# robustrobotics/multi_view_stereonet

Hardware: AMD Instinct MI355X
Metric: depthmaps/sec at 512x256, 64 hypotheses, 2 src views; L1 vs ref (higher is better)
Workload: dtype f32; 1 GPU; GTA-SfM-shaped 512x256, D=64 hypotheses, 2 source views, cost-volume filter + 5 refiners; global_batch=256, parallelism=dp1 (independent images, all-gather of metric rows)

## Files before the change

### include/mvsn_hip.h

```cpp
#ifndef MVSN_HIP_H
#define MVSN_HIP_H

#include <stddef.h>
#include <stdint.h>

#ifdef __cplusplus
extern "C" {
#endif

#define MVSN_ABI_VERSION 6

#define MVSN_E_BADARG (-1)
#define MVSN_E_TOOLARGE (-2)
#define MVSN_E_WORKSPACE (-3)

typedef void *mvsn_stream_t;

int mvsn_abi_version(void);
const char *mvsn_last_error(void);

int mvsn_plane_sweep_setup(const float *T_right_in_left, const float *K_lvl0, const float *K_lvl4,
                           int n_chains, int rows4, int cols4, int num_idepth_samples,
                           float *idepth_samples, float *H_lvl4, float *H_inc, float *H_lvl0_plane0,
                           float *baseline, mvsn_stream_t stream);
// ... 104 lines not shown
                              long spatial, float *out, mvsn_stream_t stream);
int mvsn_groupnorm_lrelu_apply_records(const float *x, const float *records, int tiles, const float *gamma,
                                       const float *beta, const float *residual, const float *r_stats,
                                       const float *r_gamma, const float *r_beta, int n, long spatial, float *out,
                                       mvsn_stream_t stream);

int mvsn_conv_to1_supported(int rows, int cols);
int mvsn_conv_to1(const float *in, const float *weight, const float *bias, const float *prior, const float *fx,
                  int n, int depth, int rows, int cols, int kd, float *out, mvsn_stream_t stream);
int mvsn_conv_to1_volume_norm(const float *in_raw, const float *in_stats, const float *in_gamma, const float *in_beta,
                              const float *weight, const float *bias, int n, int depth, int rows, int cols, float *out,
                              mvsn_stream_t stream);
int mvsn_conv_to1_block(const float *in_raw, const float *in_stats, const float *in_gamma, const float *in_beta,
                        const float *in_residual, const float *weight, const float *bias, const float *prior,
                        const float *fx, int n, int rows, int cols, float *out, mvsn_stream_t stream);
int mvsn_conv_to1_block_records(const float *in_raw, const float *in_records, int tiles, const float *in_gamma,
                                const float *in_beta, const float *in_residual, const float *weight, const float *bias,
                                const float *prior, const float *fx, int n, int rows, int cols, float *out,
                                mvsn_stream_t stream);

int mvsn_soft_argmin(const float *cost, const float *idepth_samples, int n, int num_idepth_samples,
                     int pixels, float *idepth, mvsn_stream_t stream);

int mvsn_soft_argmin_confidence(const float *cost, const float *idepth_samples, int n, int num_idepth_samples,
                                int pixels, float *idepth, float *confidence, mvsn_stream_t stream);
int mvsn_confidence_fuse_sources(const float *confidence, int n_sources, int batch, int pixels, float *out,
                                 mvsn_stream_t stream);
int mvsn_confidence_mask(const float *confidence, const uint8_t *valid, long count, float min_confidence,
                         uint8_t *out, mvsn_stream_t stream);
int mvsn_fusion_gather(const float *maps, const int *view, const int *pixel, int n_views, long pixels_per_view,
                       long count, float *out, mvsn_stream_t stream);

int mvsn_channel_l2_norm(const float *x, int n, int channels, long pixels, float *out, mvsn_stream_t stream);
int mvsn_idepth_scale(const float *prior, const float *fx, int n, long pixels, float *out, mvsn_stream_t stream);
int mvsn_refiner_epilogue(const float *prior, const float *fx, const float *delta, int n, long pixels, float *out,
                          mvsn_stream_t stream);

int mvsn_upsample_bilinear(const float *in, int n, int channels, int rows_in, int cols_in, int rows_out,
                           int cols_out, float *out, mvsn_stream_t stream);
int mvsn_upsample_prior(const float *in, const float *fx, int n, int rows_in, int cols_in, int rows_out, int cols_out,
                        float *out, float *out_scaled, mvsn_stream_t stream);
int mvsn_upsample_mask(const uint8_t *in, int n, int channels, int rows_in, int cols_in, int rows_out,
                       int cols_out, uint8_t *out, mvsn_stream_t stream);

int mvsn_area_downsample(const float *in, int n, int channels, int rows_in, int cols_in, float *out,
                         mvsn_stream_t stream);

int mvsn_image_pyramid_supported(int rows, int cols, int levels);
int mvsn_image_pyramid(const float *in, int n, int channels, int rows, int cols, int levels, float *const *out_levels,
                       mvsn_stream_t stream);
int mvsn_prepare_cameras(const float *K, const float *T_right_in_left, int batch, int n_sources, int levels,
                         const int *level_sizes_dev, float *K_pyr, float *T_normalised, float *T_inverse_normalised,
                         float *baseline, mvsn_stream_t stream);

int mvsn_fuse_sources(const float *raw, const float *refined, const float *baseline, const uint8_t *mask,
                      int n_sources, int batch, int num_idepth_samples, int pixels, int refined_aliases_raw,
                      float *raw_out, float *refined_out, uint8_t *mask_out, mvsn_stream_t stream);

int mvsn_idepth_reproject_blocks(int pixels);
int mvsn_idepth_reproject(const float *K, const float *T_other_in_this, const float *idepth, const float *other_idepth,
                          const uint8_t *other_mask, int batch, int rows, int cols, float *idepth_in_other,
                          float *other_sampled, uint8_t *other_mask_sampled, uint8_t *invalid, float *uv,
                          float *absdiff_partials, mvsn_stream_t stream);
int mvsn_occlusion_mask(const float *idepth_in_other, const float *other_sampled, const uint8_t *invalid,
                        const float *absdiff_partials, int batch, int pixels, uint8_t *mask, mvsn_stream_t stream);
int mvsn_masked_l1(const float *a, const float *b, const uint8_t *skip_a, const uint8_t *skip_b, long n, int accumulate,
                   float *loss, mvsn_stream_t stream);

typedef struct {
  const float *in[3];
  int channels[3], sample_mod[3];
  const float *block_scale;
  int scale_mod, scale_block;
  int head_chunks, n_blocks;
  int dilation[6];
  const float *weights, *params;
  int tail_mode;
  const float *prior, *fx;
  int fx_mod;
  float *out;
} mvsn_tower_desc;
int mvsn_tower_16x32(const mvsn_tower_desc *desc, int n_samples, mvsn_stream_t stream);

int mvsn_depth_metrics_blocks(long pixels);
int mvsn_depth_metrics(const float *idepth_est, const float *depth_true, const float *baseline, int batch, long pixels,
                       float min_depth, float max_depth, double *partials, double *rows, mvsn_stream_t stream);

size_t mvsn_fusion_workspace_bytes(int n_ref, int n_slots, int rows, int cols);
int mvsn_fusion_consistency(const float *depth, const uint8_t *valid, const float *K, const float *T_cam_in_world,
                            const int *ref_views, const int *neighbours, int n_views, int n_ref, int n_slots, int rows,
                            int cols, float max_reproj_px, float max_rel_depth, int min_consistent, float *fused_depth,
                            uint8_t *count, int64_t *total, void *workspace, size_t workspace_bytes,
                            mvsn_stream_t stream);
int mvsn_fusion_emit(const float *fused_depth, const float *images, const int *ref_views, int n_ref, int rows, int cols,
                     int n_slots, const void *workspace, size_t workspace_bytes, long capacity, float *points,
                     uint8_t *colors, int *view, int *pixel, mvsn_stream_t stream);

#define MVSN_VOXEL_STATUS_RANGE 1
#define MVSN_VOXEL_STATUS_TABLE 2
size_t mvsn_voxel_workspace_bytes(long n);
int mvsn_voxel_assign(const float *points, long n, float voxel_size, float inv_voxel_size, float origin_x,
                      float origin_y, float origin_z, int64_t *result, void *workspace, size_t workspace_bytes,
                      mvsn_stream_t stream);
int mvsn_voxel_merge(const float *points, const uint8_t *colors, long n, float voxel_size, float inv_voxel_size,
                     float origin_x, float origin_y, float origin_z, void *workspace, size_t workspace_bytes,
                     long capacity, void *accumulators, float *out_points, uint8_t *out_colors, int *count,
                     int64_t *first, int64_t *inverse, mvsn_stream_t stream);

int mvsn_depth_normals(const float *depth, const uint8_t *valid, const float *K, const float *T_cam_in_world,
                       int n_views, int rows, int cols, float max_rel_step, float *normals, mvsn_stream_t stream);
int mvsn_normals_gather(const float *normals, const int *view, const int *pixel, int n_views, long pixels_per_view,
                        long count, float *out, mvsn_stream_t stream);
int mvsn_voxel_normals(const float *normals, const int64_t *inverse, long n, long m, void *accumulators, float *out,
                       mvsn_stream_t stream);

#define MVSN_CLOUD_STATUS_RANGE 1
#define MVSN_CLOUD_STATUS_TABLE 2
size_t mvsn_cloud_workspace_bytes(long n_target);
int mvsn_cloud_index_build(const float *target, long n, float cell, float inv_cell, int64_t *status, void *workspace,
                           size_t workspace_bytes, mvsn_stream_t stream);
int mvsn_cloud_nearest(const float *query, long nq, float inv_cell, float r2, const void *workspace,
                       size_t workspace_bytes, long n_target, float *dist2, int64_t *index, int *within,
                       mvsn_stream_t stream);

int mvsn_tsdf_camera_batch(void);
int mvsn_tsdf_integrate(const float *depth, const uint8_t *valid, const float *weights, const float *images,
                        const float *K, const float *T_cam_in_world, int n_views, int rows, int cols, int nx, int ny,
                        int nz, float voxel_size, float origin_x, float origin_y, float origin_z, float trunc,
                        float min_depth, float *sdf_sum, float *weight, float *color_sum, mvsn_stream_t stream);
size_t mvsn_tsdf_workspace_bytes(int nx, int ny, int nz);
int mvsn_tsdf_classify(const float *sdf_sum, const float *weight, int nx, int ny, int nz, float min_weight,
                       int64_t *result, void *workspace, size_t workspace_bytes, mvsn_stream_t stream);
int mvsn_tsdf_extract(const float *sdf_sum, const float *weight, const float *color_sum, int nx, int ny, int nz,
                      float voxel_size, float origin_x, float origin_y, float origin_z, float min_weight,
                      const void *workspace, size_t workspace_bytes, long n_vertices, long n_quads, float *vertices,
                      float *normals, uint8_t *colors, int64_t *faces, int64_t *cell, mvsn_stream_t stream);

size_t mvsn_tsdf_raycast_workspace_bytes(int nx, int ny, int nz);
int mvsn_tsdf_raycast(const float *sdf_sum, const float *weight, const float *color_sum, int nx, int ny, int nz,
                      float voxel_size, float origin_x, float origin_y, float origin_z, const float *K,
                      const float *T_cam_in_world, int n_views, int rows, int cols, float min_weight, float min_depth,
                      float max_depth, float step, void *workspace, size_t workspace_bytes, float *depth,
                      float *normals, float *colors, float *weight_out, mvsn_stream_t stream);

int mvsn_copy(void *dst, const void *src, size_t nbytes, mvsn_stream_t stream);
int mvsn_copy_many(void *const *dst, const void *const *src, const size_t *nbytes, int count, mvsn_stream_t stream);
int mvsn_gather_focal(const float *const *K_pyr, int levels, int batch, float *fx, mvsn_stream_t stream);
int mvsn_gather_strided(const float *src, int count, long stride, float *dst, mvsn_stream_t stream);

int mvsn_debug_set_band_flags(int flags);

int mvsn_debug_set_wino_rowphase(int mode);

int mvsn_debug_wino_plan(const mvsn_conv_desc *desc, int carrying, int out[8]);

int mvsn_debug_conv_plan(const mvsn_conv_desc *desc, int mode, int out[8]);

int mvsn_selftest_mfma(mvsn_stream_t stream);

#ifdef __cplusplus
}
#endif
#endif
```

### multi_view_stereonet_amd/_native.py

```python
import ctypes
import os
from ctypes import c_char_p, c_int, c_long, c_size_t, c_void_p, POINTER, Structure

import torch

_LIB_PATH = os.path.join(os.path.dirname(os.path.abspath(__file__)), "libmvsn_hip.so")
_lib = None


class ConvDesc(Structure):
    _fields_ = [("n", c_int), ("c_in", c_int), ("c_out", c_int), ("depth", c_int), ("rows", c_int),
                ("cols", c_int), ("kd", c_int), ("kh", c_int), ("kw", c_int), ("stride", c_int),
                ("dilation", c_int), ("precision", c_int)]


class ApplyJob(Structure):
    _fields_ = [("x", c_void_p), ("stats", c_void_p), ("gamma", c_void_p), ("beta", c_void_p),
                ("residual", c_void_p), ("r_stats", c_void_p), ("r_gamma", c_void_p), ("r_beta", c_void_p),
                ("out", c_void_p), ("n", c_int), ("reverse", c_int), ("spatial", c_long)]


class TowerDesc(Structure):
    _fields_ = [("inp", c_void_p * 3), ("channels", c_int * 3), ("sample_mod", c_int * 3), ("block_scale", c_void_p),
                ("scale_mod", c_int), ("scale_block", c_int), ("head_chunks", c_int), ("n_blocks", c_int),
                ("dilation", c_int * 6), ("weights", c_void_p), ("params", c_void_p), ("tail_mode", c_int),
                ("prior", c_void_p), ("fx", c_void_p), ("fx_mod", c_int), ("out", c_void_p)]


CONV_FP32, CONV_BF16X3, CONV_FP32_WINO, CONV_BF16 = 0, 1, 2, 3
CHAIN_AUTO, CHAIN_DIRECT, CHAIN_WINOGRAD, CHAIN_STEPWISE, CHAIN_BANDED = 0, 1, 2, 3, 4
ABI_VERSION = 6


SIGNATURES = {
    "mvsn_abi_version": (c_int, []),
    "mvsn_last_error": (c_char_p, []),
    "mvsn_plane_sweep_setup": (c_int, [c_void_p] * 3 + [c_int] * 4 + [c_void_p] * 5 + [c_void_p]),
    "mvsn_plane_sweep_setup_sources": (c_int, [POINTER(c_void_p), c_int, c_void_p, c_void_p] + [c_int] * 4 + [c_void_p] * 5 + [c_void_p]),
    "mvsn_plane_sweep_setup_path": (c_int, [c_void_p, c_void_p, c_int, c_int]),
    "mvsn_gather_focal": (c_int, [POINTER(c_void_p), c_int, c_int, c_void_p, c_void_p]),
    "mvsn_homography_warp": (c_int, [c_void_p] * 2 + [c_int] * 5 + [c_void_p] * 2 + [c_void_p]),
    "mvsn_feature_refiner_packed_floats": (c_size_t, []),
    "mvsn_pack_feature_refiner": (c_int, [c_void_p] * 11 + [c_void_p]),
    "mvsn_incremental_cost_volume_workspace_bytes": (c_size_t, [c_int] * 3),
    "mvsn_incremental_cost_volume_form": (c_int, [c_int] * 2),
    "mvsn_incremental_cost_volume_form_for": (c_int, [c_int] * 3),
    "mvsn_incremental_cost_volume_workspace_bytes_for": (c_size_t, [c_int] * 5),
    "mvsn_incremental_cost_volume_resolve": (c_int, [c_int] * 7 + [POINTER(c_size_t * 8)]),
    "mvsn_incremental_cost_volume_status_offset": (c_size_t, [c_int] * 3),
    "mvsn_incremental_cost_volume_banded_groups": (c_int, [c_int] * 3),
    "mvsn_incremental_cost_volume": (c_int, [c_void_p] * 6 + [c_int] * 5 + [c_void_p] * 4 + [c_size_t, c_int, c_void_p]),
    "mvsn_incremental_cost_volume_repair_workspace_bytes": (c_size_t, [c_int] * 3),
    "mvsn_incremental_cost_volume_guarded": (c_int, [c_void_p] * 6 + [c_int] * 5 + [c_void_p] * 4 +
                                             [c_size_t, c_int, c_void_p, c_size_t, c_void_p, c_void_p]),
    "mvsn_incremental_cost_volume_bf16": (c_int, [c_void_p] * 6 + [c_int] * 5 + [c_void_p] * 4 +
                                          [c_size_t, c_int, c_void_p, c_size_t, c_void_p, c_void_p]),
    "mvsn_conv_bf16x3_supported": (c_int, [POINTER(ConvDesc)]),
    "mvsn_conv_forward_bf16_storage": (c_int, [c_void_p, c_void_p, c_int, c_void_p, c_void_p, c_void_p, c_void_p, c_void_p,
                                               c_void_p, c_int, c_void_p, c_void_p]),
    "mvsn_conv_winograd_supported": (c_int, [POINTER(ConvDesc)]),
    "mvsn_conv_packed_floats": (c_size_t, [POINTER(ConvDesc)]),
    "mvsn_conv_pack_weights": (c_int, [POINTER(ConvDesc), c_void_p, c_void_p, c_void_p]),
    "mvsn_conv_num_tiles": (c_int, [POINTER(ConvDesc)]),
    "mvsn_conv_forward": (c_int, [POINTER(ConvDesc)] + [c_void_p] * 10 + [c_void_p]),
    "mvsn_conv_forward_blocks": (c_int, [POINTER(ConvDesc), c_void_p, POINTER(c_int), c_int] + [c_void_p] * 4 + [c_void_p]),
    "mvsn_conv_forward_carry": (c_int, [POINTER(ConvDesc)] + [c_void_p] * 8 + [POINTER(ApplyJob), POINTER(c_int), c_void_p]),
    "mvsn_groupnorm_finalize": (c_int, [c_void_p, c_int, c_int, c_void_p, c_void_p]),
    "mvsn_groupnorm_finalize_split_workspace_bytes": (c_size_t, [c_int, c_int]),
    "mvsn_groupnorm_finalize_split": (c_int, [c_void_p, c_int, c_int, c_void_p, c_void_p, c_size_t, c_void_p]),
    "mvsn_groupnorm_lrelu_apply": (c_int, [c_void_p] * 5 + [c_int, c_long, c_void_p, c_void_p]),
    "mvsn_groupnorm_lrelu_add2": (c_int, [c_void_p] * 8 + [c_int, c_long, c_void_p, c_void_p]),
    "mvsn_conv_to1_block": (c_int, [c_void_p] * 9 + [c_int] * 3 + [c_void_p, c_void_p]),
    "mvsn_debug_set_band_flags": (c_int, [c_int]),
    "mvsn_debug_set_wino_rowphase": (c_int, [c_int]),
    "mvsn_debug_wino_plan": (c_int, [POINTER(ConvDesc), c_int, POINTER(c_int * 8)]),
    "mvsn_debug_conv_plan": (c_int, [POINTER(ConvDesc), c_int, POINTER(c_int * 8)]),
    "mvsn_copy_many": (c_int, [c_void_p, c_void_p, c_void_p, c_int, c_void_p]),
    "mvsn_conv_to1_block_records": (c_int, [c_void_p] * 2 + [c_int] + [c_void_p] * 7 + [c_int] * 3 + [c_void_p, c_void_p]),
    "mvsn_groupnorm_lrelu_apply_records": (c_int, [c_void_p] * 2 + [c_int] + [c_void_p] * 6 + [c_int, c_long, c_void_p, c_void_p]),
    "mvsn_conv_to1_supported": (c_int, [c_int, c_int]),
    "mvsn_conv_to1_volume_norm": (c_int, [c_void_p] * 6 + [c_int] * 4 + [c_void_p, c_void_p]),
    "mvsn_conv_to1": (c_int, [c_void_p] * 5 + [c_int] * 5 + [c_void_p, c_void_p]),
    "mvsn_soft_argmin": (c_int, [c_void_p] * 2 + [c_int] * 3 + [c_void_p, c_void_p]),
    "mvsn_soft_argmin_confidence": (c_int, [c_void_p] * 2 + [c_int] * 3 + [c_void_p] * 2 + [c_void_p]),
    "mvsn_confidence_fuse_sources": (c_int, [c_void_p] + [c_int] * 3 + [c_void_p, c_void_p]),
    "mvsn_confidence_mask": (c_int, [c_void_p, c_void_p, c_long, ctypes.c_float, c_void_p, c_void_p]),
    "mvsn_fusion_gather": (c_int, [c_void_p] * 3 + [c_int, c_long, c_long, c_void_p, c_void_p]),
    "mvsn_channel_l2_norm": (c_int, [c_void_p, c_int, c_int, c_long, c_void_p, c_void_p]),
    "mvsn_idepth_scale": (c_int, [c_void_p, c_void_p, c_int, c_long, c_void_p, c_void_p]),
    "mvsn_refiner_epilogue": (c_int, [c_void_p, c_void_p, c_void_p, c_int, c_long, c_void_p, c_void_p]),
    "mvsn_upsample_bilinear": (c_int, [c_void_p] + [c_int] * 6 + [c_void_p, c_void_p]),
    "mvsn_upsample_prior": (c_int, [c_void_p, c_void_p] + [c_int] * 5 + [c_void_p] * 3),
    "mvsn_upsample_mask": (c_int, [c_void_p] + [c_int] * 6 + [c_void_p, c_void_p]),
    "mvsn_image_pyramid_supported": (c_int, [c_int] * 3),
    "mvsn_image_pyramid": (c_int, [c_void_p] + [c_int] * 5 + [POINTER(c_void_p), c_void_p]),
    "mvsn_prepare_cameras": (c_int, [c_void_p] * 2 + [c_int] * 3 + [c_void_p] * 5 + [c_void_p]),
    "mvsn_area_downsample": (c_int, [c_void_p] + [c_int] * 4 + [c_void_p, c_void_p]),
    "mvsn_fuse_sources": (c_int, [c_void_p] * 4 + [c_int] * 5 + [c_void_p] * 3 + [c_void_p]),
    "mvsn_idepth_reproject_blocks": (c_int, [c_int]),
    "mvsn_idepth_reproject": (c_int, [c_void_p] * 5 + [c_int] * 3 + [c_void_p] * 6 + [c_void_p]),
    "mvsn_occlusion_mask": (c_int, [c_void_p] * 4 + [c_int] * 2 + [c_void_p, c_void_p]),
    "mvsn_masked_l1": (c_int, [c_void_p] * 4 + [c_long, c_int, c_void_p, c_void_p]),
    "mvsn_tower_16x32": (c_int, [POINTER(TowerDesc), c_int, c_void_p]),
    "mvsn_depth_metrics_blocks": (c_int, [c_long]),
    "mvsn_depth_metrics": (c_int, [c_void_p] * 3 + [c_int, c_long, ctypes.c_float, ctypes.c_float, c_void_p, c_void_p, c_void_p]),
    "mvsn_fusion_workspace_bytes": (c_size_t, [c_int] * 4),
    "mvsn_fusion_consistency": (c_int, [c_void_p] * 6 + [c_int] * 5 + [ctypes.c_float] * 2 + [c_int] + [c_void_p] * 4 +
                                [c_size_t, c_void_p]),
    "mvsn_fusion_emit": (c_int, [c_void_p] * 3 + [c_int] * 4 + [c_void_p, c_size_t, c_long] + [c_void_p] * 4 + [c_void_p]),
    "mvsn_voxel_workspace_bytes": (c_size_t, [c_long]),
    "mvsn_voxel_assign": (c_int, [c_void_p, c_long] + [ctypes.c_float] * 5 + [c_void_p, c_void_p, c_size_t, c_void_p]),
    "mvsn_voxel_merge": (c_int, [c_void_p, c_void_p, c_long] + [ctypes.c_float] * 5 + [c_void_p, c_size_t, c_long] +
                         [c_void_p] * 6 + [c_void_p]),
    "mvsn_depth_normals": (c_int, [c_void_p] * 4 + [c_int] * 3 + [ctypes.c_float, c_void_p, c_void_p]),
    "mvsn_normals_gather": (c_int, [c_void_p] * 3 + [c_int, c_long, c_long, c_void_p, c_void_p]),
    "mvsn_voxel_normals": (c_int, [c_void_p, c_void_p, c_long, c_long, c_void_p, c_void_p, c_void_p]),
    "mvsn_cloud_workspace_bytes": (c_size_t, [c_long]),
    "mvsn_cloud_index_build": (c_int, [c_void_p, c_long] + [ctypes.c_float] * 2 + [c_void_p, c_void_p, c_size_t, c_void_p]),
    "mvsn_cloud_nearest": (c_int, [c_void_p, c_long] + [ctypes.c_float] * 2 + [c_void_p, c_size_t, c_long] +
                           [c_void_p] * 3 + [c_void_p]),
    "mvsn_tsdf_camera_batch": (c_int, []),
    "mvsn_tsdf_integrate": (c_int, [c_void_p] * 6 + [c_int] * 6 + [ctypes.c_float] * 6 + [c_void_p] * 3 + [c_void_p]),
    "mvsn_tsdf_workspace_bytes": (c_size_t, [c_int] * 3),
    "mvsn_tsdf_classify": (c_int, [c_void_p] * 2 + [c_int] * 3 + [ctypes.c_float, c_void_p, c_void_p, c_size_t, c_void_p]),
    "mvsn_tsdf_extract": (c_int, [c_void_p] * 3 + [c_int] * 3 + [ctypes.c_float] * 5 + [c_void_p, c_size_t, c_long, c_long] +
                          [c_void_p] * 5 + [c_void_p]),
    "mvsn_tsdf_raycast_workspace_bytes": (c_size_t, [c_int] * 3),
    "mvsn_tsdf_raycast": (c_int, [c_void_p] * 3 + [c_int] * 3 + [ctypes.c_float] * 4 + [c_void_p] * 2 + [c_int] * 3 +
                          [ctypes.c_float] * 4 + [c_void_p, c_size_t] + [c_void_p] * 4 + [c_void_p]),
    "mvsn_copy": (c_int, [c_void_p, c_void_p, c_size_t, c_void_p]),
    "mvsn_gather_strided": (c_int, [c_void_p, c_int, c_long, c_void_p, c_void_p]),
    "mvsn_selftest_mfma": (c_int, [c_void_p]),
}


def library_path() -> str:
    return _LIB_PATH


def load():
    global _lib
    if _lib is not None:
        return _lib
    if not os.path.exists(_LIB_PATH):
        raise RuntimeError(
            f"{_LIB_PATH} is missing: the HIP extension has not been built "
            "(run `python -m multi_view_stereonet_amd.build` or __graft_entry__.build()). "
            "There is no CPU fallback for the plane-sweep path.")
    lib = ctypes.CDLL(_LIB_PATH)
    lib.mvsn_abi_version.restype, lib.mvsn_abi_version.argtypes = c_int, []
    if lib.mvsn_abi_version() != ABI_VERSION:
        raise RuntimeError(f"libmvsn_hip.so is ABI version {lib.mvsn_abi_version()}, this package needs {ABI_VERSION}: "
                           "rebuild it (python -m multi_view_stereonet_amd.build --force)")
    for name, (res, args) in SIGNATURES.items():
        fn = getattr(lib, name)
        fn.restype = res
        fn.argtypes = args
    _lib = lib
    return lib


def ptr(t):
    if t is None:
        return None
    if not t.is_cuda:
        raise RuntimeError("libmvsn_hip.so takes device (HBM) pointers; got a CPU tensor")
    if not t.is_contiguous():
        raise RuntimeError("libmvsn_hip.so takes dense tensors")
    return t.data_ptr()


def stream():
    return torch.cuda.current_stream().cuda_stream


def plane_sweep_setup_path(K_lvl0, K_lvl4, rows4: int, cols4: int):
    lib = load()
    K0, K4 = (k.detach().to("cpu", torch.float32).contiguous() for k in (K_lvl0, K_lvl4))
    return [lib.mvsn_plane_sweep_setup_path(K0[n].data_ptr(), K4[n].data_ptr(), rows4, cols4) for n in range(K0.shape[0])]


def check(rc: int, what: str):
    if rc != 0:
        msg = load().mvsn_last_error()
        raise RuntimeError(f"{what} failed (code {rc}): {msg.decode() if msg else ''}")


_coresident = {}


def _device_key(index: int) -> str:
    p = torch.cuda.get_device_properties(index)
    uuid = getattr(p, "uuid", None)
    if uuid is not None and str(uuid).strip("0-") != "":
        return str(uuid)
    return "pci-%04x-%02x-%02x" % (getattr(p, "pci_domain_id", 0), getattr(p, "pci_bus_id", index),
                                   getattr(p, "pci_device_id", 0))


def coresident_lock_path(index: int) -> str:
    root = os.environ.get("MVSN_LOCK_DIR") or "/tmp"
    return os.path.join(root, "mvsn_coresident_%s.lock" % _device_key(index).replace("/", "_"))


def coresident_right(index: int) -> bool:
    if index in _coresident:
        return _coresident[index][0]
    if os.environ.get("MVSN_CORESIDENT_LOCK", "1") == "0":
        _coresident[index] = (True, None)
        return True
    import fcntl
    try:
        old_mask = os.umask(0)
        try:
            f = os.fdopen(os.open(coresident_lock_path(index), os.O_RDWR | os.O_CREAT, 0o666), "r+")
        finally:
            os.umask(old_mask)
    except OSError:
        _coresident[index] = (True, None)
        return True
    try:
        fcntl.flock(f, fcntl.LOCK_EX | fcntl.LOCK_NB)
    except OSError:
        f.close()
        _coresident[index] = (False, None)
        return False
    try:
# ... 16 lines not shown
```

### multi_view_stereonet_amd/csrc/mvsn_misc.hip

```cpp
#include <type_traits>

#include "mvsn_geom.h"
#include "mvsn_resident.h"

namespace mvsn {

__global__ __launch_bounds__(256) void soft_argmin_kernel(const float *__restrict__ cost,
                                                          const float *__restrict__ samples, int D, int P,
                                                          float *__restrict__ out) {
  const int p = blockIdx.x * blockDim.x + threadIdx.x;
  const int n = blockIdx.y;
  if (p >= P) return;
  const float *c = cost + (size_t)n * D * P + p;
  const float *s = samples + (size_t)n * D;
  float m = -INFINITY;
  int d0 = 0;
  for (; d0 + 16 <= D; d0 += 16) {
    float v[16];
#pragma unroll
    for (int j = 0; j < 16; ++j) v[j] = c[(size_t)(d0 + j) * P];
#pragma unroll
    for (int j = 0; j < 16; ++j) m = fmaxf(m, -v[j]);
  }
  for (int d = d0; d < D; ++d) m = fmaxf(m, -c[(size_t)d * P]);
// ... 539 lines not shown
        for (int t = 0; t < 2; ++t)
#pragma unroll
          for (int r = 0; r < 4; ++r) {
            const int tap = t * 16 + (lane >> 4) * 4 + r;
            if (tap < 27)
              *reinterpret_cast<floatx4 *>(P + tap * T3_SLOTS + s0) = floatx4{d[t][0][r], d[t][1][r], d[t][2][r], d[t][3][r]};
          }
      }
    }
  };

  for (int z = zb - 1; z <= ze; ++z) {
    if (z >= 0 && z < D) {
      plane_products(z);
      lds_barrier();
#pragma unroll
      for (int dz = 0; dz < 3; ++dz)
#pragma unroll
        for (int dy = 0; dy < 3; ++dy)
#pragma unroll
          for (int dx = 0; dx < 3; ++dx) {
            const float *q = pg + (dz * 9 + dy * 3 + dx) * T3_SLOTS + dy * T3_XS + dx;
            acc[2 - dz][0] += q[0];
            acc[2 - dz][1] += q[1];
          }
    }
    if (z - 1 >= zb && z - 1 < ze && o_ok) {
      float2 v = make_float2(acc[0][0] + b, acc[0][1] + b);
      *reinterpret_cast<float2 *>(outn + (size_t)(z - 1) * plane) = v;
    }
    acc[0][0] = acc[1][0], acc[0][1] = acc[1][1];
    acc[1][0] = acc[2][0], acc[1][1] = acc[2][1];
    acc[2][0] = 0.f, acc[2][1] = 0.f;
    lds_barrier();
  }
}

constexpr int T2_TY = 16;
template <int TX>
struct T2 {
  static constexpr int XS = TX + 8, SLOTS = (T2_TY + 2) * XS, GROUPS = (SLOTS + 63) / 64, LDS_FLOATS = 9 * SLOTS;
};
static inline bool to1_wide_tiles(int n, int rows, int cols) {
  return (long)n * ((rows + T2_TY - 1) / T2_TY) * ((cols + 63) / 64) >= 4L * device_cus();
}

template <bool XFORM, int T2_TX>
__global__ __launch_bounds__(256) void conv_to1_2d_mfma_kernel(const float *__restrict__ in, const float *__restrict__ w,
                                                               const float *__restrict__ bias,
                                                               const float *__restrict__ in_stats,
                                                               const float *__restrict__ in_gamma,
                                                               const float *__restrict__ in_beta,
                                                               const float *__restrict__ in_residual,
                                                               const float *__restrict__ prior, const float *__restrict__ fx,
                                                               int H, int W, int ntx, int stat_tiles,
                                                               float *__restrict__ out) {
  constexpr int T2_XS = T2<T2_TX>::XS, T2_SLOTS = T2<T2_TX>::SLOTS, T2_GROUPS = T2<T2_TX>::GROUPS;
  __shared__ __attribute__((aligned(16))) float P[T2<T2_TX>::LDS_FLOATS];
  const int tid = threadIdx.x, lane = tid & 63;
  const int wave = __builtin_amdgcn_readfirstlane(tid >> 6);
  const int n = blockIdx.y;
  const int tile = xcd_tile_index(blockIdx.x, gridDim.x);
  const int tyi = tile / ntx, txi = tile - tyi * ntx;
  const int y0 = tyi * T2_TY, x0 = txi * T2_TX;
  const size_t plane = (size_t)H * W;
  const int kc = lane >> 4;
  const float *inn = in + ((size_t)n * 32 + kc) * plane;
  const float *resn = (XFORM && in_residual) ? in_residual + ((size_t)n * 32 + kc) * plane : nullptr;

  float a[8];
  float sc[8], sh[8];
  __shared__ float gst[8];
  const float *st = nullptr;
  if constexpr (XFORM) st = gn_stats_here(in_stats, stat_tiles, n, gst);
#pragma unroll
  for (int ks = 0; ks < 8; ++ks) {
    const int tap = lane & 15, c = ks * 4 + kc;
    a[ks] = tap < 9 ? w[c * 9 + tap] : 0.0f;
    if constexpr (XFORM) {
      const float mean = st[(c >> 3) * 2 + 0];
      const float rstd = st[(c >> 3) * 2 + 1];
      sc[ks] = rstd * in_gamma[c];
      sh[ks] = in_beta[c] - mean * sc[ks];
    }
  }

  constexpr int GPW = (T2_GROUPS + 3) / 4;
#pragma unroll
  for (int u = 0; u < GPW; ++u) {
    if ((wave + 4 * u) * 64 >= T2_SLOTS) break;
    const int s0 = (wave + 4 * u) * 64 + 4 * (lane & 15);
    const int row = s0 / T2_XS, col = s0 - row * T2_XS;
    const int gy = y0 - 1 + row, gx = x0 - 4 + col;
    const bool ok = s0 < T2_SLOTS && gy >= 0 && gy < H && gx >= 0 && gx < W;
    const size_t off = ok ? (size_t)gy * W + gx : 0;
    floatx4 bfr[8], rfr[8];
#pragma unroll
    for (int ks = 0; ks < 8; ++ks) {
      bfr[ks] = ok ? *reinterpret_cast<const floatx4 *>(inn + (size_t)ks * 4 * plane + off) : floatx4{0.f, 0.f, 0.f, 0.f};
      if constexpr (XFORM)
        rfr[ks] = (ok && resn) ? *reinterpret_cast<const floatx4 *>(resn + (size_t)ks * 4 * plane + off)
                               : floatx4{0.f, 0.f, 0.f, 0.f};
    }
    floatx4 d[4];
#pragma unroll
    for (int p = 0; p < 4; ++p) d[p] = floatx4{0.f, 0.f, 0.f, 0.f};
#pragma unroll
    for (int ks = 0; ks < 8; ++ks) {
      if constexpr (XFORM) {
        const float shk = ok ? sh[ks] : 0.0f;
#pragma unroll
        for (int p = 0; p < 4; ++p) bfr[ks][p] = rfr[ks][p] + lrelu02(bfr[ks][p] * sc[ks] + shk);
      }
#pragma unroll
      for (int p = 0; p < 4; ++p) d[p] = mfma16x16x4(a[ks], bfr[ks][p], d[p]);
    }
    if (s0 < T2_SLOTS) {
#pragma unroll
      for (int r = 0; r < 4; ++r) {
        const int tap = kc * 4 + r;
        if (tap < 9) *reinterpret_cast<floatx4 *>(P + tap * T2_SLOTS + s0) = floatx4{d[0][r], d[1][r], d[2][r], d[3][r]};
      }
    }
  }
  __syncthreads();
  const float b = bias ? bias[0] : 0.0f;
#pragma unroll
  for (int k = 0; k < T2_TY * T2_TX / 512; ++k) {
    const int idx = tid + 256 * k;
    const int oy = idx / (T2_TX / 2), ox = (idx % (T2_TX / 2)) * 2;
    if (y0 + oy >= H || x0 + ox >= W) continue;
    const float *pg = P + oy * T2_XS + ox + 3;
    float acc0 = 0.f, acc1 = 0.f;
#pragma unroll
    for (int dy = 0; dy < 3; ++dy)
#pragma unroll
      for (int dx = 0; dx < 3; ++dx) {
        const float *q = pg + (dy * 3 + dx) * T2_SLOTS + dy * T2_XS + dx;
        acc0 += q[0];
        acc1 += q[1];
      }
    const size_t o = (size_t)n * plane + (size_t)(y0 + oy) * W + x0 + ox;
    float2 res = make_float2(acc0 + b, acc1 + b);
    if (prior) {
      const float g = fx[n];
      const float2 pv = *reinterpret_cast<const float2 *>(prior + o);
      const float s0v = pv.x * g + res.x, s1v = pv.y * g + res.y;
      res = make_float2(relu_nan(s0v) / g, relu_nan(s1v) / g);
    }
    *reinterpret_cast<float2 *>(out + o) = res;
  }
}

}

static int conv_to1_volume(const float *in, const float *weight, const float *bias, const float *in_stats,
                           const float *in_gamma, const float *in_beta, int n, int depth, int rows, int cols,
                           float *out, mvsn_stream_t stream) {
  using namespace mvsn;
  const int nty = (rows + T3_TY - 1) / T3_TY, ntx = (cols + T3_TX - 1) / T3_TX;
  int nslab = 1;
  while (nslab < 8 && (long)n * nty * ntx * nslab < 1024 && depth / (nslab * 2) >= 8) nslab *= 2;
  while (nslab < depth && (long)n * nty * ntx * nslab * 2 <= device_cus()) nslab *= 2;
  const int zslab = (depth + nslab - 1) / nslab;
  const int nz = (depth + zslab - 1) / zslab;
  MVSN_REQUIRE(n <= 65535 && nz <= 65535, MVSN_E_TOOLARGE, "mvsn_conv_to1: grid");
  const size_t lds = (size_t)T3_LDS_FLOATS * sizeof(float);
  const bool whole = rows == T3_TY && cols == T3_TX;
#define MVSN_TO1_3D_LAUNCH(XF_, WHOLE_)                                                                                \
  do {                                                                                                                 \
    static LdsOptIn opt;                                                                                               \
    if (int rc = ensure_lds(opt, (const void *)conv_to1_3d_mfma_kernel<XF_, WHOLE_>, lds, "mvsn_conv_to1")) return rc; \
    hipLaunchKernelGGL((conv_to1_3d_mfma_kernel<XF_, WHOLE_>), dim3(nty * ntx, nz, n), dim3(256), lds,                 \
                       (hipStream_t)stream, in, weight, bias, in_stats, in_gamma, in_beta, depth, rows, cols, ntx,     \
                       zslab, out);                                                                                    \
  } while (0)
  if (in_stats) {
    if (whole) MVSN_TO1_3D_LAUNCH(true, true);
    else MVSN_TO1_3D_LAUNCH(true, false);
  } else {
    in_gamma = in_beta = nullptr;
    if (whole) MVSN_TO1_3D_LAUNCH(false, true);
    else MVSN_TO1_3D_LAUNCH(false, false);
  }
#undef MVSN_TO1_3D_LAUNCH
  return mvsn::check_launch("mvsn_conv_to1(volume)");
}

extern "C" int mvsn_conv_to1_supported(int rows, int cols) { return (cols % 4 == 0 && rows > 0) ? 1 : 0; }

extern "C" int mvsn_conv_to1(const float *in, const float *weight, const float *bias, const float *prior,
                             const float *fx, int n, int depth, int rows, int cols, int kd, float *out,
                             mvsn_stream_t stream) {
  MVSN_REQUIRE(in && weight && out, MVSN_E_BADARG, "mvsn_conv_to1: null pointer");
  MVSN_REQUIRE(n > 0 && depth > 0 && rows > 0 && cols > 0 && (kd == 1 || kd == 3), MVSN_E_BADARG,
               "mvsn_conv_to1: bad sizes");
  MVSN_REQUIRE(cols % 4 == 0, MVSN_E_BADARG, "mvsn_conv_to1: cols must be a multiple of 4 (use mvsn_conv_forward)");
  MVSN_REQUIRE(!prior || (fx && depth == 1), MVSN_E_BADARG, "mvsn_conv_to1: refiner epilogue needs fx and 2-D input");
  if (kd == 3) {
    return conv_to1_volume(in, weight, bias, nullptr, nullptr, nullptr, n, depth, rows, cols, out, stream);
  } else {
    MVSN_REQUIRE(depth == 1, MVSN_E_BADARG, "mvsn_conv_to1: kd = 1 needs depth = 1");
    MVSN_REQUIRE(n <= 65535, MVSN_E_TOOLARGE, "mvsn_conv_to1: grid");
    const int nty = (rows + mvsn::T2_TY - 1) / mvsn::T2_TY;
    if (mvsn::to1_wide_tiles(n, rows, cols)) {
      const int ntx = (cols + 63) / 64;
      hipLaunchKernelGGL((mvsn::conv_to1_2d_mfma_kernel<false, 64>), dim3(nty * ntx, n), dim3(256), 0,
                         (hipStream_t)stream, in, weight, bias, (const float *)nullptr, (const float *)nullptr,
                         (const float *)nullptr, (const float *)nullptr, prior, fx, rows, cols, ntx, 0, out);
    } else {
      const int ntx = (cols + 31) / 32;
      hipLaunchKernelGGL((mvsn::conv_to1_2d_mfma_kernel<false, 32>), dim3(nty * ntx, n), dim3(256), 0,
                         (hipStream_t)stream, in, weight, bias, (const float *)nullptr, (const float *)nullptr,
                         (const float *)nullptr, (const float *)nullptr, prior, fx, rows, cols, ntx, 0, out);
    }
  }
  return mvsn::check_launch("mvsn_conv_to1");
}

extern "C" int mvsn_conv_to1_volume_norm(const float *in_raw, const float *in_stats, const float *in_gamma,
                                         const float *in_beta, const float *weight, const float *bias, int n, int depth,
                                         int rows, int cols, float *out, mvsn_stream_t stream) {
  MVSN_REQUIRE(in_raw && in_stats && in_gamma && in_beta && weight && out, MVSN_E_BADARG,
               "mvsn_conv_to1_volume_norm: null pointer");
  MVSN_REQUIRE(n > 0 && depth > 0 && rows > 0 && cols > 0, MVSN_E_BADARG, "mvsn_conv_to1_volume_norm: bad sizes");
  MVSN_REQUIRE(cols % 4 == 0, MVSN_E_BADARG, "mvsn_conv_to1_volume_norm: cols must be a multiple of 4");
  return conv_to1_volume(in_raw, weight, bias, in_stats, in_gamma, in_beta, n, depth, rows, cols, out, stream);
}

static int conv_to1_block_launch(const char *what, const float *in_raw, const float *in_stats, int stat_tiles,
                                 const float *in_gamma, const float *in_beta, const float *in_residual,
                                 const float *weight, const float *bias, const float *prior, const float *fx, int n,
                                 int rows, int cols, float *out, mvsn_stream_t stream) {
  MVSN_REQUIRE(in_raw && in_stats && in_gamma && in_beta && weight && out, MVSN_E_BADARG, "%s: null pointer", what);
  MVSN_REQUIRE(n > 0 && rows > 0 && cols > 0, MVSN_E_BADARG, "%s: bad sizes", what);
  MVSN_REQUIRE(cols % 4 == 0, MVSN_E_BADARG, "%s: cols must be a multiple of 4", what);
  MVSN_REQUIRE(!prior || fx, MVSN_E_BADARG, "%s: refiner epilogue needs fx", what);
  MVSN_REQUIRE(n <= 65535, MVSN_E_TOOLARGE, "%s: grid", what);
  const int nty = (rows + mvsn::T2_TY - 1) / mvsn::T2_TY;
  if (mvsn::to1_wide_tiles(n, rows, cols)) {
    const int ntx = (cols + 63) / 64;
    hipLaunchKernelGGL((mvsn::conv_to1_2d_mfma_kernel<true, 64>), dim3(nty * ntx, n), dim3(256), 0, (hipStream_t)stream,
                       in_raw, weight, bias, in_stats, in_gamma, in_beta, in_residual, prior, fx, rows, cols, ntx,
                       stat_tiles, out);
  } else {
    const int ntx = (cols + 31) / 32;
    hipLaunchKernelGGL((mvsn::conv_to1_2d_mfma_kernel<true, 32>), dim3(nty * ntx, n), dim3(256), 0, (hipStream_t)stream,
                       in_raw, weight, bias, in_stats, in_gamma, in_beta, in_residual, prior, fx, rows, cols, ntx,
                       stat_tiles, out);
  }
  return mvsn::check_launch(what);
}

extern "C" int mvsn_conv_to1_block(const float *in_raw, const float *in_stats, const float *in_gamma,
                                   const float *in_beta, const float *in_residual, const float *weight,
                                   const float *bias, const float *prior, const float *fx, int n, int rows, int cols,
                                   float *out, mvsn_stream_t stream) {
  return conv_to1_block_launch("mvsn_conv_to1_block", in_raw, in_stats, 0, in_gamma, in_beta, in_residual, weight, bias,
                               prior, fx, n, rows, cols, out, stream);
}

extern "C" int mvsn_conv_to1_block_records(const float *in_raw, const float *in_records, int tiles,
                                           const float *in_gamma, const float *in_beta, const float *in_residual,
                                           const float *weight, const float *bias, const float *prior, const float *fx,
                                           int n, int rows, int cols, float *out, mvsn_stream_t stream) {
  MVSN_REQUIRE(tiles > 0, MVSN_E_BADARG, "mvsn_conv_to1_block_records: tiles");
  return conv_to1_block_launch("mvsn_conv_to1_block_records", in_raw, in_records, tiles, in_gamma, in_beta, in_residual,
                               weight, bias, prior, fx, n, rows, cols, out, stream);
}

namespace mvsn {

__global__ __launch_bounds__(256) void soft_argmin_confidence_kernel(const float *__restrict__ cost,
                                                                     const float *__restrict__ samples, int D, int P,
                                                                     float *__restrict__ out,
                                                                     float *__restrict__ confidence) {
  const int p = blockIdx.x * blockDim.x + threadIdx.x;
  const int n = blockIdx.y;
  if (p >= P) return;
  const float *c = cost + (size_t)n * D * P + p;
  const float *s = samples + (size_t)n * D;
  float m = -INFINITY;
  int d0 = 0;
  for (; d0 + 16 <= D; d0 += 16) {
    float v[16];
#pragma unroll
    for (int j = 0; j < 16; ++j) v[j] = c[(size_t)(d0 + j) * P];
#pragma unroll
    for (int j = 0; j < 16; ++j) m = fmaxf(m, -v[j]);
  }
  for (int d = d0; d < D; ++d) m = fmaxf(m, -c[(size_t)d * P]);
  float den = 0.0f, num = 0.0f, idx = 0.0f;
  for (d0 = 0; d0 + 16 <= D; d0 += 16) {
    float v[16];
#pragma unroll
    for (int j = 0; j < 16; ++j) v[j] = c[(size_t)(d0 + j) * P];
#pragma unroll
    for (int j = 0; j < 16; ++j) {
      const float e = expf(-v[j] - m);
      den += e;
      num += e * s[d0 + j];
      idx += e * (float)(d0 + j);
    }
  }
  for (int d = d0; d < D; ++d) {
    float e = expf(-c[(size_t)d * P] - m);
    den += e;
    num += e * s[d];
    idx += e * (float)d;
  }
  out[(size_t)n * P + p] = num / den;
  const float expected = idx / den;
  float conf = NAN;
  if (expected == expected) {
    int i = (int)floorf(expected);
    i = i < 0 ? 0 : (i > D - 1 ? D - 1 : i);
    float w[4];
#pragma unroll
    for (int k = 0; k < 4; ++k) {
      const int d = i - 1 + k;
      const bool in = d >= 0 && d < D;
      w[k] = in ? c[(size_t)(in ? d : 0) * P] : INFINITY;
    }
    float sum = 0.0f;
#pragma unroll
    for (int k = 0; k < 4; ++k) sum += expf(-w[k] - m);
    conf = sum / den;
  }
  confidence[(size_t)n * P + p] = conf;
}

__global__ __launch_bounds__(256) void confidence_fuse_kernel(const float *__restrict__ conf, int S, int B, int P,
                                                              float *__restrict__ out) {
  const int p = blockIdx.x * blockDim.x + threadIdx.x;
  const int b = blockIdx.y;
  if (p >= P) return;
  float acc = conf[(size_t)b * P + p];
  for (int s = 1; s < S; ++s) {
    const float v = conf[((size_t)s * B + b) * P + p];
    acc = (v != v || v < acc) ? v : acc;
  }
  out[(size_t)b * P + p] = acc;
}

__global__ __launch_bounds__(256) void confidence_mask_kernel(const float *__restrict__ conf,
                                                              const uint8_t *__restrict__ valid, long count, float thr,
                                                              uint8_t *__restrict__ out) {
  const long i = (long)blockIdx.x * blockDim.x + threadIdx.x;
  if (i >= count) return;
  const bool keep = conf[i] >= thr && (valid == nullptr || valid[i] != 0);
  out[i] = keep ? 1 : 0;
}

}

extern "C" int mvsn_soft_argmin_confidence(const float *cost, const float *idepth_samples, int n, int D, int pixels,
                                           float *idepth, float *confidence, mvsn_stream_t stream) {
  MVSN_REQUIRE(cost && idepth_samples && idepth && confidence, MVSN_E_BADARG, "mvsn_soft_argmin_confidence: null pointer");
  MVSN_REQUIRE(n > 0 && D > 0 && pixels > 0 && n <= 65535, MVSN_E_BADARG, "mvsn_soft_argmin_confidence: bad sizes");
  hipLaunchKernelGGL(mvsn::soft_argmin_confidence_kernel, dim3((pixels + 255) / 256, n), dim3(256), 0,
                     (hipStream_t)stream, cost, idepth_samples, D, pixels, idepth, confidence);
  return mvsn::check_launch("mvsn_soft_argmin_confidence");
}

extern "C" int mvsn_confidence_fuse_sources(const float *confidence, int n_sources, int batch, int pixels, float *out,
                                            mvsn_stream_t stream) {
  MVSN_REQUIRE(confidence && out, MVSN_E_BADARG, "mvsn_confidence_fuse_sources: null pointer");
  MVSN_REQUIRE(n_sources > 0 && batch > 0 && batch <= 65535 && pixels > 0, MVSN_E_BADARG,
               "mvsn_confidence_fuse_sources: bad sizes");
  hipLaunchKernelGGL(mvsn::confidence_fuse_kernel, dim3((pixels + 255) / 256, batch), dim3(256), 0, (hipStream_t)stream,
                     confidence, n_sources, batch, pixels, out);
  return mvsn::check_launch("mvsn_confidence_fuse_sources");
}

extern "C" int mvsn_confidence_mask(const float *confidence, const uint8_t *valid, long count, float min_confidence,
                                    uint8_t *out, mvsn_stream_t stream) {
  MVSN_REQUIRE(confidence && out, MVSN_E_BADARG, "mvsn_confidence_mask: null pointer");
  MVSN_REQUIRE(count > 0 && (count + 255) / 256 <= 2147483647L, MVSN_E_BADARG, "mvsn_confidence_mask: bad sizes");
  MVSN_REQUIRE(min_confidence == min_confidence, MVSN_E_BADARG, "mvsn_confidence_mask: the threshold is NaN");
  hipLaunchKernelGGL(mvsn::confidence_mask_kernel, dim3((unsigned)((count + 255) / 256)), dim3(256), 0,
                     (hipStream_t)stream, confidence, valid, count, min_confidence, out);
  return mvsn::check_launch("mvsn_confidence_mask");
}

extern "C" int mvsn_fusion_gather(const float *maps, const int *view, const int *pixel, int n_views, long pixels_per_view,
                                  long count, float *out, mvsn_stream_t stream) {
  MVSN_REQUIRE(maps && view && pixel && out, MVSN_E_BADARG, "mvsn_fusion_gather: null pointer");
  MVSN_REQUIRE(n_views > 0 && pixels_per_view > 0 && pixels_per_view <= 2147483647L && count > 0 &&
                   (count + 255) / 256 <= 2147483647L,
               MVSN_E_BADARG, "mvsn_fusion_gather: bad sizes");
  hipLaunchKernelGGL(mvsn::gather_kernel<1>, dim3((unsigned)((count + 255) / 256)), dim3(256), 0, (hipStream_t)stream,
                     maps, view, pixel, n_views, pixels_per_view, count, out);
  return mvsn::check_launch("mvsn_fusion_gather");
// ... 2 lines not shown
```

Baseline: 3836 depthmaps/s.

## Add row-strip conv_to1 kernel that walks column tiles with register double-buffering

```diff
diff --git a/include/mvsn_hip.h b/include/mvsn_hip.h
--- a/include/mvsn_hip.h
+++ b/include/mvsn_hip.h
@@ -280,6 +280,9 @@
 
 int mvsn_debug_set_wino_rowphase(int mode);
 
+int mvsn_debug_set_to1_strip(int mode);
+int mvsn_debug_to1_plan(int n, int rows, int cols);
+
 int mvsn_debug_wino_plan(const mvsn_conv_desc *desc, int carrying, int out[8]);
 
 int mvsn_debug_conv_plan(const mvsn_conv_desc *desc, int mode, int out[8]);
diff --git a/multi_view_stereonet_amd/_native.py b/multi_view_stereonet_amd/_native.py
--- a/multi_view_stereonet_amd/_native.py
+++ b/multi_view_stereonet_amd/_native.py
@@ -73,6 +73,8 @@
     "mvsn_conv_to1_block": (c_int, [c_void_p] * 9 + [c_int] * 3 + [c_void_p, c_void_p]),
     "mvsn_debug_set_band_flags": (c_int, [c_int]),
     "mvsn_debug_set_wino_rowphase": (c_int, [c_int]),
+    "mvsn_debug_set_to1_strip": (c_int, [c_int]),
+    "mvsn_debug_to1_plan": (c_int, [c_int] * 3),
     "mvsn_debug_wino_plan": (c_int, [POINTER(ConvDesc), c_int, POINTER(c_int * 8)]),
     "mvsn_debug_conv_plan": (c_int, [POINTER(ConvDesc), c_int, POINTER(c_int * 8)]),
     "mvsn_copy_many": (c_int, [c_void_p, c_void_p, c_void_p, c_int, c_void_p]),
diff --git a/multi_view_stereonet_amd/csrc/mvsn_misc.hip b/multi_view_stereonet_amd/csrc/mvsn_misc.hip
--- a/multi_view_stereonet_amd/csrc/mvsn_misc.hip
+++ b/multi_view_stereonet_amd/csrc/mvsn_misc.hip
@@ -715,6 +715,186 @@
   }
 }
 
+template <bool XFORM>
+__global__ __launch_bounds__(256, 2) void conv_to1_2d_strip_kernel(const float *__restrict__ in, const float *__restrict__ w,
+                                                                const float *__restrict__ bias,
+                                                                const float *__restrict__ in_stats,
+                                                                const float *__restrict__ in_gamma,
+                                                                const float *__restrict__ in_beta,
+                                                                const float *__restrict__ in_residual,
+                                                                const float *__restrict__ prior, const float *__restrict__ fx,
+                                                                int H, int W, int ntx, int stat_tiles,
+                                                                float *__restrict__ out) {
+  constexpr int TX = 64, XS = T2<TX>::XS, SLOTS = T2<TX>::SLOTS, ROWS = T2_TY + 2, ROUNDS = (ROWS + 3) / 4;
+  __shared__ __attribute__((aligned(16))) float P[T2<TX>::LDS_FLOATS];
+  const int tid = threadIdx.x, lane = tid & 63;
+  const int wave = __builtin_amdgcn_readfirstlane(tid >> 6);
+  const int n = blockIdx.y;
+  const int y0 = xcd_tile_index(blockIdx.x, gridDim.x) * T2_TY;
+  const size_t plane = (size_t)H * W;
+  const int kc = lane >> 4, li = lane & 15;
+  const unsigned sample_bytes = (unsigned)(32 * plane * 4);
+  const __amdgpu_buffer_rsrc_t rin =
+      __builtin_amdgcn_make_buffer_rsrc(const_cast<float *>(in + (size_t)n * 32 * plane), 0, (int)sample_bytes, 0x00020000);
+  const bool has_res = XFORM && in_residual;
+  const __amdgpu_buffer_rsrc_t rres = __builtin_amdgcn_make_buffer_rsrc(
+      const_cast<float *>(has_res ? in_residual + (size_t)n * 32 * plane : in), 0, has_res ? (int)sample_bytes : 0, 0x00020000);
+  const int kstep_bytes = (int)(16 * plane);
+
+  float a[8];
+  float sc[8], sh[8];
+  __shared__ float gst[8];
+  const float *st = nullptr;
+  if constexpr (XFORM) st = gn_stats_here(in_stats, stat_tiles, n, gst);
+#pragma unroll
+  for (int ks = 0; ks < 8; ++ks) {
+    const int tap = lane & 15, c = ks * 4 + kc;
+    a[ks] = tap < 9 ? w[c * 9 + tap] : 0.0f;
+    if constexpr (XFORM) {
+      const float mean = st[(c >> 3) * 2 + 0];
+      const float rstd = st[(c >> 3) * 2 + 1];
+      sc[ks] = rstd * in_gamma[c];
+      sh[ks] = in_beta[c] - mean * sc[ks];
+    }
+  }
+
+  const bool carrier = tid < 9 * ROWS;
+  float *const cp = P + (carrier ? (tid / ROWS) * SLOTS + (tid % ROWS) * XS : 0);
+  if (carrier) {
+    *reinterpret_cast<floatx4 *>(cp) = floatx4{0.f, 0.f, 0.f, 0.f};
+    *reinterpret_cast<floatx4 *>(cp + TX + 4) = floatx4{0.f, 0.f, 0.f, 0.f};
+  }
+
+  auto load_round = [&](int k, int j, floatx4 (&bfr)[8], floatx4 (&rfr)[8]) -> bool {
+    const int row = wave + 4 * j, gy = y0 - 1 + row, gx = k * TX + 4 * li;
+    const bool ok = k < ntx && row < ROWS && gy >= 0 && gy < H && gx < W;
+    const unsigned off = ok ? ((unsigned)kc * (unsigned)plane + (unsigned)gy * W + gx) * 4u : 0x80000000u;
+#pragma unroll
+    for (int ks = 0; ks < 8; ++ks) {
+      bfr[ks] = __builtin_bit_cast(floatx4, __builtin_amdgcn_raw_buffer_load_b128(rin, off, ks * kstep_bytes, 0));
+      if constexpr (XFORM)
+        rfr[ks] = __builtin_bit_cast(floatx4, __builtin_amdgcn_raw_buffer_load_b128(rres, off, ks * kstep_bytes, 0));
+    }
+    return ok;
+  };
+  auto round_products = [&](int j, bool ok, floatx4 (&bfr)[8], floatx4 (&rfr)[8]) {
+    const int row = wave + 4 * j;
+    if (row >= ROWS) return;
+    floatx4 d[4];
+#pragma unroll
+    for (int p = 0; p < 4; ++p) d[p] = floatx4{0.f, 0.f, 0.f, 0.f};
+#pragma unroll
+    for (int ks = 0; ks < 8; ++ks) {
+      if constexpr (XFORM) {
+        const float shk = ok ? sh[ks] : 0.0f;
+#pragma unroll
+        for (int p = 0; p < 4; ++p) bfr[ks][p] = rfr[ks][p] + lrelu02(bfr[ks][p] * sc[ks] + shk);
+      }
+#pragma unroll
+      for (int p = 0; p < 4; ++p) d[p] = mfma16x16x4(a[ks], bfr[ks][p], d[p]);
+    }
+#pragma unroll
+    for (int r = 0; r < 4; ++r) {
+      const int tap = kc * 4 + r;
+      if (tap < 9)
+        *reinterpret_cast<floatx4 *>(P + tap * SLOTS + row * XS + 4 + 4 * li) = floatx4{d[0][r], d[1][r], d[2][r], d[3][r]};
+    }
+  };
+  const float b = bias ? bias[0] : 0.0f;
+  const float g = prior ? fx[n] : 1.0f;
+  const __amdgpu_buffer_rsrc_t rprior = __builtin_amdgcn_make_buffer_rsrc(
+      const_cast<float *>(prior ? prior + (size_t)n * plane : in), 0, prior ? (int)(plane * 4) : 0, 0x00020000);
+  constexpr unsigned NO_OUTPUT = 0x80000000u;
+  auto out_offset = [&](int x0, int oy, int ox) -> unsigned {
+    return (y0 + oy < H && x0 + ox >= 0 && x0 + ox < W) ? ((unsigned)(y0 + oy) * W + x0 + ox) * 4u : NO_OUTPUT;
+  };
+  auto load_prior = [&](unsigned ooff) -> float2 {
+    return make_float2(__builtin_bit_cast(float, __builtin_amdgcn_raw_buffer_load_b32(rprior, ooff, 0, 0)),
+                       __builtin_bit_cast(float, __builtin_amdgcn_raw_buffer_load_b32(rprior, ooff + 4, 0, 0)));
+  };
+  auto emit = [&](unsigned ooff, int oy, int ox, float2 pv) {
+    if (ooff == NO_OUTPUT) return;
+    const float *pg = P + oy * XS + ox + 3;
+    float acc0 = 0.f, acc1 = 0.f;
+#pragma unroll
+    for (int dy = 0; dy < 3; ++dy)
+#pragma unroll
+      for (int dx = 0; dx < 3; ++dx) {
+        const float *q = pg + (dy * 3 + dx) * SLOTS + dy * XS + dx;
+        acc0 += q[0];
+        acc1 += q[1];
+      }
+    float2 res = make_float2(acc0 + b, acc1 + b);
+    if (prior) {
+      const float s0v = pv.x * g + res.x, s1v = pv.y * g + res.y;
+      res = make_float2(relu_nan(s0v) / g, relu_nan(s1v) / g);
+    }
+    *reinterpret_cast<float2 *>(out + (size_t)n * plane + (ooff >> 2)) = res;
+  };
+
+  floatx4 bfA[8], rfA[8], bfB[8], rfB[8];
+  bool okA = load_round(0, 0, bfA, rfA), okB = false;
+  auto tile = [&](int k, bool &okc, floatx4 (&bfc)[8], floatx4 (&rfc)[8], bool &okn, floatx4 (&bfn)[8], floatx4 (&rfn)[8]) {
+    static_assert(ROUNDS == 5, "an odd number of rounds: the tile loop below alternates the register sets");
+    constexpr int PAIRS = T2_TY * TX / 512;
+    const int x0 = k * TX;
+    unsigned ooff[PAIRS + 1];
+    float2 pv[PAIRS + 1];
+#pragma unroll
+    for (int kk = 0; kk < PAIRS; ++kk) {
+      const int idx = tid + 256 * kk;
+      ooff[kk] = out_offset(x0, idx / (TX / 2), (idx % (TX / 2)) * 2 - 2);
+    }
+    ooff[PAIRS] = (k == ntx - 1 && tid < T2_TY) ? out_offset(x0, tid, TX - 2) : NO_OUTPUT;
+#pragma unroll
+    for (int kk = 0; kk <= PAIRS; ++kk) pv[kk] = load_prior(ooff[kk]);
+#pragma unroll
+    for (int j = 0; j < ROUNDS; ++j) {
+      const int nk = j + 1 < ROUNDS ? k : k + 1, nj = j + 1 < ROUNDS ? j + 1 : 0;
+      if ((j & 1) == 0) {
+        okn = load_round(nk, nj, bfn, rfn);
+        round_products(j, okc, bfc, rfc);
+      } else {
+        okc = load_round(nk, nj, bfc, rfc);
+        round_products(j, okn, bfn, rfn);
+      }
+    }
+    lds_barrier();
+#pragma unroll
+    for (int kk = 0; kk < PAIRS; ++kk) {
+      const int idx = tid + 256 * kk;
+      emit(ooff[kk], idx / (TX / 2), (idx % (TX / 2)) * 2 - 2, pv[kk]);
+    }
+    emit(ooff[PAIRS], tid & (T2_TY - 1), TX - 2, pv[PAIRS]);
+    floatx4 cv = floatx4{0.f, 0.f, 0.f, 0.f};
+    if (carrier) cv = *reinterpret_cast<const floatx4 *>(cp + TX);
+    lds_barrier();
+    if (carrier) *reinterpret_cast<floatx4 *>(cp) = cv;
+  };
+  for (int k = 0; k < ntx; k += 2) {
+    tile(k, okA, bfA, rfA, okB, bfB, rfB);
+    if (k + 1 < ntx) tile(k + 1, okB, bfB, rfB, okA, bfA, rfA);
+  }
+}
+
+static int g_to1_strip = 0;
+static inline bool to1_strips(int n, int rows, int cols) {
+  if ((long)rows * cols >= (1L << 24)) return false;
+  if (g_to1_strip != 0) return g_to1_strip == 1;
+  return to1_wide_tiles(n, rows, cols) && (long)n * ((rows + T2_TY - 1) / T2_TY) >= 2L * device_cus();
+}
+
+}
+
+extern "C" int mvsn_debug_set_to1_strip(int mode) {
+  const int old = mvsn::g_to1_strip;
+  mvsn::g_to1_strip = mode;
+  return old;
+}
+
+extern "C" int mvsn_debug_to1_plan(int n, int rows, int cols) {
+  if (n <= 0 || rows <= 0 || cols <= 0 || cols % 4 != 0) return -1;
+  return mvsn::to1_strips(n, rows, cols) ? 2 : mvsn::to1_wide_tiles(n, rows, cols) ? 1 : 0;
 }
 
 static int conv_to1_volume(const float *in, const float *weight, const float *bias, const float *in_stats,
@@ -766,7 +946,12 @@
     MVSN_REQUIRE(depth == 1, MVSN_E_BADARG, "mvsn_conv_to1: kd = 1 needs depth = 1");
     MVSN_REQUIRE(n <= 65535, MVSN_E_TOOLARGE, "mvsn_conv_to1: grid");
     const int nty = (rows + mvsn::T2_TY - 1) / mvsn::T2_TY;
-    if (mvsn::to1_wide_tiles(n, rows, cols)) {
+    if (mvsn::to1_strips(n, rows, cols)) {
+      MVSN_REQUIRE(nty <= 65535, MVSN_E_TOOLARGE, "mvsn_conv_to1: grid");
+      hipLaunchKernelGGL((mvsn::conv_to1_2d_strip_kernel<false>), dim3(nty, n), dim3(256), 0, (hipStream_t)stream, in,
+                         weight, bias, (const float *)nullptr, (const float *)nullptr, (const float *)nullptr,
+                         (const float *)nullptr, prior, fx, rows, cols, (cols + 63) / 64, 0, out);
+    } else if (mvsn::to1_wide_tiles(n, rows, cols)) {
       const int ntx = (cols + 63) / 64;
       hipLaunchKernelGGL((mvsn::conv_to1_2d_mfma_kernel<false, 64>), dim3(nty * ntx, n), dim3(256), 0,
                          (hipStream_t)stream, in, weight, bias, (const float *)nullptr, (const float *)nullptr,
@@ -801,7 +986,12 @@
   MVSN_REQUIRE(!prior || fx, MVSN_E_BADARG, "%s: refiner epilogue needs fx", what);
   MVSN_REQUIRE(n <= 65535, MVSN_E_TOOLARGE, "%s: grid", what);
   const int nty = (rows + mvsn::T2_TY - 1) / mvsn::T2_TY;
-  if (mvsn::to1_wide_tiles(n, rows, cols)) {
+  if (mvsn::to1_strips(n, rows, cols)) {
+    MVSN_REQUIRE(nty <= 65535, MVSN_E_TOOLARGE, "%s: grid", what);
+    hipLaunchKernelGGL((mvsn::conv_to1_2d_strip_kernel<true>), dim3(nty, n), dim3(256), 0, (hipStream_t)stream, in_raw,
+                       weight, bias, in_stats, in_gamma, in_beta, in_residual, prior, fx, rows, cols, (cols + 63) / 64,
+                       stat_tiles, out);
+  } else if (mvsn::to1_wide_tiles(n, rows, cols)) {
     const int ntx = (cols + 63) / 64;
     hipLaunchKernelGGL((mvsn::conv_to1_2d_mfma_kernel<true, 64>), dim3(nty * ntx, n), dim3(256), 0, (hipStream_t)stream,
                        in_raw, weight, bias, in_stats, in_gamma, in_beta, in_residual, prior, fx, rows, cols, ntx,
```

Result: no change. 3863 depthmaps/s (median of 6 runs) (+0.7%).
